# mirage/decompress

Measured on AMD Instinct MI355X. Metric: MiB/s inflate over N zlib streams (uncompressed bytes / wall second), higher is better.
Workload: dtype u8; 1 GPU; C2: 4096 x 256 KiB zlib streams per GPU, dynamic Huffman (libz level 6; even streams = slices of the reference's test/corpus, odd = order-2 Markov ASCII text, 64 symbols, seed 0xC2 + i, SURVEY 8(d)), Zl.Inf.Ns semantics, one stream per pair of wavefronts (decoder + copier); streams_per_gpu=4096, stream_bytes=262144, unique_streams=4096

## Files before the change

decompress_amd/csrc/inflate_wave.hip:

```cpp
#include <stdlib.h>
#include "inflate_util.hpp"
#include "internal.hpp"

namespace md {
namespace wv {

constexpr uint32_t S = 264;
constexpr uint32_t SMIN = 48;
constexpr uint32_t KMAX = 64;
#ifndef MD_EMIT_SPLIT
#define MD_EMIT_SPLIT 1
#endif
#if defined(MD_DEBUG_KNOWN_BOUNDS)
#undef MD_EMIT_SPLIT
#define MD_EMIT_SPLIT 0
#endif
#ifndef MD_SPLIT_B
#define MD_SPLIT_B 4
#endif
#ifndef MD_RUNIN_NUM
#define MD_RUNIN_NUM 3
#define MD_RUNIN_DEN 2
#endif
constexpr uint32_t RUNIN_NUM = MD_RUNIN_NUM, RUNIN_DEN = MD_RUNIN_DEN;
constexpr uint32_t PASSES = 5;
constexpr uint32_t PASS_BITS = 1600, PASSES_MAX = 16;
#ifndef MD_RMAX
#define MD_RMAX 576
#endif
#ifndef MD_STAGE
#define MD_STAGE 5248
#endif
#ifndef MD_PAIR_OCC
#define MD_PAIR_OCC 5
#endif
constexpr uint32_t RMAX = MD_RMAX;
constexpr uint32_t STAGE = MD_STAGE;
constexpr uint32_t WIN_WORDS = 544;

constexpr uint32_t kLitSize = 852, kDistSize = 592;
constexpr uint32_t kLitRootMax = 512;
constexpr uint32_t kLitSubB = 0;
constexpr uint32_t kDistB = kLitSize - kLitRootMax;
constexpr uint32_t kLitB = kDistB + kDistSize;
constexpr uint32_t kStopEobI = kLitB + kLitRootMax;
constexpr uint32_t kStopBadI = kStopEobI + 2;
constexpr uint32_t kLutWords = kStopBadI + 2;
constexpr uint32_t kTbMask = 0xffe00000u;
constexpr uint32_t kLoopy = 0x100u;
static_assert(kDistB % 2 == 0 && kLitB % 2 == 0 && kStopEobI % 2 == 0 && kLutWords == 1448, "even table bases");
constexpr uint32_t kStEob = 100, kStTrunc = 101;
constexpr uint32_t kCountMatch = 1u << 20;
constexpr uint32_t kNearBit = 0x8000u;

struct Mail {
  uint32_t emitted;
  uint32_t copied;
  uint32_t kind;
  uint32_t total;
  uint32_t x;
  uint32_t stuck;
  uint32_t a, b;
};
constexpr uint32_t kJobRound = 0, kJobStored = 1, kJobQuit = 2, kJobEmit = 3;
constexpr uint32_t kHxUni = 4 * 64;
struct Smem {
  uint32_t win[WIN_WORDS];
  uint32_t lut[kLutWords];
  uint32_t mrec[RMAX];
  uint16_t mpos[RMAX];
  alignas(16) uint8_t stage[STAGE + 16];
  uint16_t list[RMAX];
  Mail mail;
};
struct HScratch {
  uint8_t lens[384];
  uint16_t work[320];
  uint32_t ctr;
};
#if MD_RMAX == 576 && MD_STAGE == 5248
static_assert(sizeof(Smem) <= 17920, "9 streams (18 wavefronts) per CU: 160 KiB / 9, in whole 512-byte units");
#endif
static_assert(RMAX % 64 == 0 && STAGE % 16 == 0 && RMAX * 2 >= (kHxUni + 6) * 4, "record rows, staging chunks, the emit job's words in `list`");
constexpr uint32_t kHScratchAt = 1136;
static_assert(kHScratchAt >= 4 + 572 + 8 && kHScratchAt % 16 == 0 && kHScratchAt + sizeof(HScratch) <= WIN_WORDS * 4, "header scratch lives behind the header's bits");
typedef MD_LDS Smem lds_smem;
typedef MD_LDS HScratch lds_hscratch;
__device__ __forceinline__ lds_hscratch *hscratch_of(lds_smem *sm) {
  return reinterpret_cast<lds_hscratch *>(reinterpret_cast<lds_u8 *>(sm->win) + kHScratchAt);
}

#ifdef MD_DEBUG_KNOWN_BOUNDS
constexpr uint32_t KB_ROUNDS = 512;
__device__ uint4 *g_kb_buf;
__device__ int g_kb_mode;
#endif
__device__ __forceinline__ uint32_t mk_entry(uint32_t n, uint32_t xb, uint32_t val8, uint32_t nbits, uint32_t tb) {
  return n | (xb << 5) | (val8 << 9) | (nbits << 17) | (tb << 21);
}
__device__ __forceinline__ uint32_t e_n(uint32_t e) { return e & 31; }
__device__ __forceinline__ uint32_t e_xb(uint32_t e) { return (e >> 5) & 15; }
__device__ __forceinline__ uint32_t e_val(uint32_t e) { return (e >> 9) & 255; }
__device__ __forceinline__ uint32_t e_tb(uint32_t e) { return e >> 21; }
__device__ __forceinline__ bool e_link(uint32_t e) { return e_tb(e) < kLitB && e_tb(e) != kDistB; }
__device__ __forceinline__ uint32_t e_root(uint32_t lroot) { return mk_entry(0, 0, 0, lroot, kLitB); }
__device__ __forceinline__ uint32_t lit_leaf(uint32_t sym, uint32_t codelen, uint32_t lroot, uint32_t droot) {
  if (sym < 256) return mk_entry(codelen, 0, sym, lroot, kLitB);
  if (sym == 256) return mk_entry(codelen, 0, 0, 0, kStopEobI);
  const uint32_t l = (sym - 257) & 31;
  const uint32_t xb = (l >= 8 && l < 28) ? (l - 4) >> 2 : 0;
  const uint32_t base3 = l < 8 ? l : l < 28 ? (4 + (l & 3)) << xb : l == 28 ? 255 : 0;
  return mk_entry(codelen + xb, xb, base3, droot, kDistB);
}
__device__ __forceinline__ uint32_t dist_leaf(uint32_t dv, uint32_t codelen, uint32_t lroot) {
  dv &= 31;
  if (dv >= 30) return mk_entry(codelen, 0, 0, 0, kStopBadI);
  const uint32_t xb = dv >= 4 ? (dv - 2) >> 1 : 0;
  const uint32_t m = dv < 4 ? dv : ((dv & 1) | 2);
  return mk_entry(codelen + xb, xb, m, lroot, kLitB);
}
__device__ __forceinline__ uint32_t dist_value(uint32_t m, uint32_t xb, uint32_t x) { return (m << xb) + 1 + x; }

struct Window {
  uint32_t w[8], wx;
  uint32_t base;
#ifdef MD_DEBUG_KNOWN_BOUNDS
  uint32_t kb_round, kb_sid;
#endif
  __device__ __forceinline__ void fetch(const uint8_t *__restrict__ body, uint32_t nbytes, uint32_t b, uint32_t lane) {
    base = b;
    const uint32_t off = b + lane * 32;
#pragma unroll
    for (int k = 0; k < 8; k++) w[k] = 0;
    if (off + 32 <= nbytes) __builtin_memcpy(w, body + off, 32);
    else if (off < nbytes)
      for (uint32_t k = 0; k < 32 && off + k < nbytes; k++) w[k >> 2] |= (uint32_t)body[off + k] << (8 * (k & 3));
    wx = 0;
    if (lane < WIN_WORDS - 512) {
      const uint32_t ox = b + 2048 + lane * 4;
      if (ox + 4 <= nbytes) __builtin_memcpy(&wx, body + ox, 4);
      else if (ox < nbytes)
        for (uint32_t k = 0; k < 4 && ox + k < nbytes; k++) wx |= (uint32_t)body[ox + k] << (8 * k);
    }
  }
  __device__ __forceinline__ void put(lds_u32 *win, uint32_t lane) const {
    lds_u32 *dst = win + lane * 8;
#pragma unroll
    for (int k = 0; k < 8; k++) dst[k] = w[k];
    if (lane < WIN_WORDS - 512) win[512 + lane] = wx;
  }
  __device__ __forceinline__ void ensure(lds_u32 *win, const uint8_t *__restrict__ body, uint32_t nbytes, uint32_t b, uint32_t lane) {
    if (base != b) fetch(body, nbytes, b, lane);
    put(win, lane);
    base = 0xffffffffu;
  }
};
__device__ __forceinline__ uint32_t peek(const lds_u32 *win, uint32_t p) {
  const lds_u32 *q = reinterpret_cast<const lds_u32 *>(reinterpret_cast<const lds_u8 *>(win) + ((p >> 3) & ~3u));
  return __builtin_amdgcn_alignbit(q[1], q[0], p & 31);
}
__device__ __forceinline__ uint32_t lut_at(const lds_u32 *lut, uint32_t tb, uint32_t idx) {
  return *reinterpret_cast<const lds_u32 *>(reinterpret_cast<const lds_u8 *>(lut) + ((tb + idx) << 2));
}

struct UBits {
  const lds_u32 *win;
  uint64_t buf;
  uint32_t n;
  uint32_t wp;
  __device__ __forceinline__ void init(const lds_u32 *w, uint32_t bp) {
    win = w;
    wp = bp >> 5;
    buf = ((uint64_t)uni(win[wp]) | ((uint64_t)uni(win[wp + 1]) << 32)) >> (bp & 31);
    n = 64 - (bp & 31);
    wp += 2;
  }
  __device__ __forceinline__ uint32_t pos() const { return wp * 32 - n; }
  __device__ __forceinline__ void fill() {
    if (n <= 32) {
      buf |= (uint64_t)uni(win[wp]) << n;
      n += 32;
      wp++;
    }
  }
  __device__ __forceinline__ uint32_t peekb(uint32_t k) const { return (uint32_t)buf & ((1u << k) - 1); }
  __device__ __forceinline__ void drop(uint32_t k) {
    buf >>= k;
    n -= k;
  }
};

struct Canon {
  uint32_t cnt[16];
  uint32_t first[16];
  uint32_t offs[16];
  uint32_t max, min, root, left;
};
__device__ __forceinline__ uint32_t lane_rank(uint64_t m) {
  return __builtin_amdgcn_mbcnt_hi((uint32_t)(m >> 32), __builtin_amdgcn_mbcnt_lo((uint32_t)m, 0));
}
template <int K>
__device__ __forceinline__ void canon_counts(const uint32_t (&len)[K], uint32_t rootpref, Canon &c) {
#pragma unroll
  for (int l = 1; l < 16; l++) {
    uint32_t n = 0;
#pragma unroll
    for (int k = 0; k < K; k++) n += (uint32_t)__builtin_popcountll(__ballot(len[k] == (uint32_t)l));
    c.cnt[l] = n;
  }
  c.cnt[0] = 0;
  c.max = 0;
  c.min = 16;
#pragma unroll
  for (int l = 15; l >= 1; l--) {
    if (c.cnt[l] && c.max == 0) c.max = l;
    if (c.cnt[l]) c.min = l;
  }
  int left = 1;
  bool over = false;
  uint32_t code = 0, off = 0;
  c.first[0] = 0;
  c.offs[0] = 0;
#pragma unroll
  for (int l = 1; l < 16; l++) {
    left = (left << 1) - (int)c.cnt[l];
    over = over || left < 0;
    code = (code + c.cnt[l - 1]) << 1;
    c.first[l] = code;
    c.offs[l] = off;
    off += c.cnt[l];
  }
  c.left = over ? 0xffffffffu : (uint32_t)left;
  uint32_t root = rootpref;
  if (root > c.max) root = c.max;
  if (root < c.min) root = c.min;
  c.root = root;
}

template <int K, class LEAF>
__device__ __forceinline__ bool build_walk(const uint32_t (&len)[K], const Canon &c, lds_u32 *lut, uint32_t tb0, uint32_t sub0,
                                           uint32_t size, lds_hscratch *hs, uint32_t lane, uint32_t zero_entry, LEAF leaf) {
  const uint32_t root = c.root, rmask = (1u << root) - 1;
  uint32_t rev[K];
#pragma unroll
  for (int k = 0; k < K; k++) rev[k] = 0;
#pragma unroll
  for (int l = 1; l < 16; l++) {
    if (c.cnt[l]) {
      uint32_t base = 0;
#pragma unroll
      for (int k = 0; k < K; k++) {
        const uint64_t m = __ballot(len[k] == (uint32_t)l);
        if (len[k] == (uint32_t)l) {
          const uint32_t rank = base + lane_rank(m);
          rev[k] = __brev(c.first[l] + rank) >> (32 - l);
          hs->work[c.offs[l] + rank] = (uint16_t)(lane + 64 * k);
        }
        base += (uint32_t)__builtin_popcountll(m);
      }
    }
  }
  const uint32_t nroot = 1u << root;
  for (uint32_t i = lane; i < nroot; i += kWave) lut[tb0 + i] = 0;
  if (lane == 0) hs->ctr = 0;
  if (c.max > root) {
#pragma unroll
    for (int k = 0; k < K; k++)
      if (len[k] > root)
        __hip_atomic_fetch_max(&lut[tb0 + (rev[k] & rmask)], len[k], __ATOMIC_RELAXED, __HIP_MEMORY_SCOPE_WORKGROUP);
  }
  for (uint32_t i = lane; i < nroot; i += kWave) {
    const uint32_t v = lut[tb0 + i];
    uint32_t e;
    if (v) {
      const uint32_t sub = v - root;
      const uint32_t off = __hip_atomic_fetch_add(&hs->ctr, 1u << sub, __ATOMIC_RELAXED, __HIP_MEMORY_SCOPE_WORKGROUP);
      e = mk_entry(root, 0, 0, sub, (sub0 + off) & 2047);
    } else {
      const uint32_t cw = __brev(i) >> (32 - root);
      uint32_t fl = 0, ft = 0;
#pragma unroll
      for (int l = 15; l >= 1; l--) {
        if (c.cnt[l] && (uint32_t)l <= root) {
          const uint32_t t = (cw >> (root - l)) - c.first[l];
          if (t < c.cnt[l]) {
            fl = l;
            ft = c.offs[l] + t;
          }
        }
      }
      e = fl ? leaf((uint32_t)hs->work[ft], fl) : zero_entry;
    }
    lut[tb0 + i] = e;
  }
  const uint32_t used = nroot + uni(hs->ctr);
  if (used > size) return false;
  if (c.max > root) {
#pragma unroll
    for (int k = 0; k < K; k++) {
      if (len[k] > root) {
        const uint32_t link = lut[tb0 + (rev[k] & rmask)];
        const uint32_t sub = (link >> 17) & 15, tb = link >> 21;
        const uint32_t e = leaf(lane + 64 * k, len[k] - root);
        for (uint32_t j = rev[k] >> root; j < (1u << sub); j += 1u << (len[k] - root)) lut[tb + j] = e;
      }
    }
  }
  return true;
}

constexpr uint64_t kZig0 = 16ull | 17ull << 5 | 18ull << 10 | 0ull << 15 | 8ull << 20 | 7ull << 25 | 9ull << 30 | 6ull << 35 |
                           10ull << 40 | 5ull << 45 | 11ull << 50 | 4ull << 55;
constexpr uint64_t kZig1 = 12ull | 3ull << 5 | 13ull << 10 | 2ull << 15 | 14ull << 20 | 1ull << 25 | 15ull << 30;

template <class PF>
__device__ __noinline__ int dynamic_tables(lds_smem *sm, uint32_t bp_arg, uint32_t tot_arg, uint32_t lane, uint32_t *bp_out,
                                           uint32_t *lroot_out, PF &pf) {
  const uint32_t bp = uni(bp_arg), tot = uni(tot_arg);
  const lds_u32 *win = (const lds_u32 *)sm->win;
  lds_hscratch *hs = hscratch_of(sm);
  UBits ub;
  ub.init(win, bp);
  if ((int32_t)(tot - ub.pos()) < 14) return MD_UNEXPECTED_END_OF_INPUT;
  const uint32_t hlit = ub.peekb(5) + 257;
  ub.drop(5);
  const uint32_t hdist = ub.peekb(5) + 1;
  ub.drop(5);
  const uint32_t hclen = ub.peekb(4) + 4;
  ub.drop(4);
  uint32_t cl[1] = {0};
  for (uint32_t i = 0; i < hclen; i++) {
    ub.fill();
    if ((int32_t)(tot - ub.pos()) < 3) return MD_UNEXPECTED_END_OF_INPUT;
    const uint32_t v = ub.peekb(3);
    ub.drop(3);
    const uint32_t z = (uint32_t)((i < 12 ? kZig0 >> (5 * i) : kZig1 >> (5 * (i - 12))) & 31);
    if (lane == z) cl[0] = v;
  }
  Canon cc;
  canon_counts<1>(cl, 7, cc);
  uint32_t cmaxl, t_lo, t_hi;
  if (cc.max == 0) {
    cmaxl = 1;
    t_lo = lane == 0 ? (1u << 8) : 0xffffu;
    t_hi = 0xffffu;
  } else {
    if (cc.left != 0) return MD_INVALID_DICTIONARY;
    cmaxl = cc.max;
#pragma unroll
    for (int l = 1; l < 8; l++) {
      const uint64_t m = __ballot(cl[0] == (uint32_t)l);
      if (cl[0] == (uint32_t)l) hs->work[cc.offs[l] + lane_rank(m)] = (uint16_t)lane;
    }
    uint32_t t[2];
#pragma unroll
    for (int h = 0; h < 2; h++) {
      const uint32_t i = lane + 64 * h;
      const uint32_t cw = __brev(i & ((1u << cmaxl) - 1)) >> (32 - cmaxl);
      uint32_t fl = 0, ft = 0;
#pragma unroll
      for (int l = 7; l >= 1; l--) {
        if (cc.cnt[l] && (uint32_t)l <= cmaxl) {
          const uint32_t x = (cw >> (cmaxl - l)) - cc.first[l];
          if (x < cc.cnt[l]) {
            fl = l;
            ft = cc.offs[l] + x;
          }
        }
      }
      t[h] = fl ? ((uint32_t)hs->work[ft] | (fl << 8)) : 0xffffu;
    }
    t_lo = t[0];
    t_hi = t[1];
  }
  const uint32_t max_res = hlit + hdist;
  for (uint32_t x = lane; x < 384; x += kWave) hs->lens[x] = 0;
  auto run_lengths = [&](auto checked) -> int {
    constexpr bool CHECK = decltype(checked)::value;
    uint32_t i = 0, prev = 0;
    while (i < max_res) {
      ub.fill();
      if (CHECK && (int32_t)(tot - ub.pos()) < (int32_t)cmaxl) return MD_UNEXPECTED_END_OF_INPUT;
      const uint32_t idx = ub.peekb(cmaxl);
      const uint32_t e_lo = __builtin_amdgcn_readlane(t_lo, idx & 63), e_hi = __builtin_amdgcn_readlane(t_hi, idx & 63);
      const uint32_t e = idx < 64 ? e_lo : e_hi;
      if (e == 0xffffu) return MD_INVALID_DICTIONARY;
      const uint32_t sym = e & 0xff;
      ub.drop(e >> 8);
      if (sym < 16) {
        hs->lens[i] = (uint8_t)sym;
        prev = sym;
        i++;
      } else {
        const uint32_t nb = sym == 16 ? 2 : sym == 17 ? 3 : 7;
        if (sym == 16 && i == 0) return MD_INVALID_DICTIONARY;
        ub.fill();
        if (CHECK && (int32_t)(tot - ub.pos()) < (int32_t)nb) return MD_UNEXPECTED_END_OF_INPUT;
        const uint32_t copy = ub.peekb(nb) + (sym == 18 ? 11 : 3);
        ub.drop(nb);
        const uint32_t val = sym == 16 ? prev : 0;
        if (i + copy > max_res) return MD_INVALID_DICTIONARY;
        if (val)
          for (uint32_t x = lane; x < copy; x += kWave) hs->lens[i + x] = (uint8_t)val;
        prev = val;
        i += copy;
      }
    }
    return MD_OK;
  };
  {
    const bool plenty = (int32_t)(tot - ub.pos()) >= 316 * 14 + 64;
    const int rc = plenty ? run_lengths(std::false_type{}) : run_lengths(std::true_type{});
    if (rc != MD_OK) return rc;
  }
  *bp_out = ub.pos();
  pf.tick_lds(P_HDR_LENS);
  if (uni(hs->lens[256]) == 0) return MD_INVALID_DICTIONARY;
  uint32_t ll[5], dl[1];
#pragma unroll
  for (int k = 0; k < 5; k++) ll[k] = lane + 64 * k < hlit ? (uint32_t)hs->lens[lane + 64 * k] : 0u;
  dl[0] = lane < hdist ? (uint32_t)hs->lens[hlit + lane] : 0u;
  Canon cl_, cd_;
  canon_counts<5>(ll, 9, cl_);
  canon_counts<1>(dl, 6, cd_);
  if (cl_.left == 0xffffffffu || (cl_.left > 0 && cl_.max != 1)) return MD_INVALID_DICTIONARY;
  const uint32_t lroot = cl_.root;
  uint32_t droot;
  lds_u32 *lut = (lds_u32 *)sm->lut;
  if (cd_.max == 0) {
    droot = 1;
  } else {
    if (cd_.left == 0xffffffffu || (cd_.left > 0 && cd_.max != 1)) return MD_INVALID_DICTIONARY;
    droot = cd_.root;
  }
  if (!build_walk<5>(ll, cl_, lut, kLitB, kLitSubB, kLitSize, hs, lane, e_root(lroot),
                     [=](uint32_t sym, uint32_t codelen) { return lit_leaf(sym, codelen, lroot, droot); }))
    return MD_INVALID_DICTIONARY;
  pf.tick_lds(P_HDR_LIT);
  if (cd_.max == 0) {
    if (lane == 0) {
      lut[kDistB] = dist_leaf(0, 1, lroot);
      lut[kDistB + 1] = mk_entry(0, 0, 0, 0, kStopBadI);
    }
  } else if (!build_walk<1>(dl, cd_, lut, kDistB, kDistB + (1u << droot), kDistSize, hs, lane, e_root(lroot),
                            [=](uint32_t sym, uint32_t codelen) { return dist_leaf(sym, codelen, lroot); }))
    return MD_INVALID_DICTIONARY;
  const bool loopy = cl_.left > 0 || (cd_.max != 0 && cd_.left > 0);
  *lroot_out = lroot | (loopy ? kLoopy : 0u);
  return MD_OK;
}

__device__ __noinline__ void fixed_tables(lds_smem *sm, uint32_t lane, uint32_t *lroot_out) {
  lds_hscratch *hs = hscratch_of(sm);
  uint32_t ll[5], dl[1];
#pragma unroll
  for (int k = 0; k < 5; k++) {
    const uint32_t n = lane + 64 * k;
    ll[k] = n < 144 ? 8 : n < 256 ? 9 : n < 280 ? 7 : n < 288 ? 8 : 0;
  }
  dl[0] = lane < 32 ? 5 : 0;
  Canon cl_, cd_;
  canon_counts<5>(ll, 9, cl_);
  canon_counts<1>(dl, 6, cd_);
  const uint32_t lroot = cl_.root, droot = cd_.root;
  lds_u32 *lut = (lds_u32 *)sm->lut;
  build_walk<5>(ll, cl_, lut, kLitB, kLitSubB, kLitSize, hs, lane, e_root(lroot),
                [=](uint32_t sym, uint32_t codelen) { return lit_leaf(sym, codelen, lroot, droot); });
  build_walk<1>(dl, cd_, lut, kDistB, kDistB + (1u << droot), kDistSize, hs, lane, e_root(lroot),
                [=](uint32_t sym, uint32_t codelen) { return dist_leaf(sym, codelen, lroot); });
  *lroot_out = lroot;
}

struct Cursor {
  uint32_t w0, w1, w2, wa;
  __device__ __forceinline__ void init(const lds_u32 *win, uint32_t p) {
    wa = (p >> 5) << 2;
    const lds_u32 *q = reinterpret_cast<const lds_u32 *>(reinterpret_cast<const lds_u8 *>(win) + wa);
    w0 = q[0];
    w1 = q[1];
    w2 = q[2];
  }
  __device__ __forceinline__ uint32_t peek(uint32_t p) const { return __builtin_amdgcn_alignbit(w1, w0, p); }
  __device__ __forceinline__ void seek(const lds_u32 *win, uint32_t pn) {
    const uint32_t wan = (pn >> 5) << 2;
    const bool ge = wan != wa;
    w0 = ge ? w1 : w0;
    w1 = ge ? w2 : w1;
    wa = wan;
    w2 = *reinterpret_cast<const lds_u32 *>(reinterpret_cast<const lds_u8 *>(win) + wa + 8);
  }
};
__device__ __forceinline__ uint32_t lut_step(const lds_u32 *lut, uint32_t e, uint32_t w) {
  return lut_at(lut, e >> 21, __builtin_amdgcn_ubfe(w, 0, e >> 17));
}

template <bool COUNT, bool BUDGET, bool MID = false>
__device__ __forceinline__ void sync_pass(const lds_u32 *win, const lds_u32 *lut, uint32_t lroot, bool go, uint32_t start,
                                          uint32_t limit, uint32_t &end, uint32_t &stop, uint32_t &nb, uint32_t mthr = 0,
                                          uint32_t *midp = nullptr, uint32_t *midcnt = nullptr) {
  if (go) {
    uint32_t p = start, e = e_root(lroot), cnt = 0;
    uint32_t mp = 0xffffffffu, mc = 0;
    bool got = false;
    if (MID && start >= mthr) {
      mp = start;
      got = true;
    }
    if (p < limit) {
      const uint32_t thr = (kLitB << 21) | limit;
      uint32_t slot = 0, key;
      Cursor c;
      c.init(win, start);
      do {
        const uint32_t w = c.peek(p);
        const uint32_t en = lut_step(lut, e, w);
        const uint32_t n = e_n(en);
        if (COUNT) {
          const uint32_t xb = e_xb(en);
          const uint32_t len1 = e_val(en) + __builtin_amdgcn_ubfe(w, n - xb, xb) + (kCountMatch + 2);
          cnt += (e_tb(en) == kLitB ? 1u : 0u) + (e_tb(en) == kDistB ? len1 : 0u);
        }
        p += n;
        if (MID) {
          const bool cross = (e_tb(en) == kLitB) & !got & (p >= mthr);
          mp = cross ? p : mp;
          mc = cross ? cnt : mc;
          got = got | cross;
        }
        c.seek(win, p);
        e = en;
        key = (en & kTbMask) | p;
        if (BUDGET && ++slot >= KMAX && e_tb(en) == kLitB) break;
      } while (key < thr);
    }
    end = p;
    stop = e_tb(e) >= kStopEobI ? e_tb(e) : 0u;
    if (COUNT) nb = cnt;
    if (MID) {
      *midp = mp;
      *midcnt = mc;
    }
  }
}

struct LaneOut {
  uint32_t endp;
  uint32_t stopc;
  uint32_t bytes;
  uint32_t nm;
};

__device__ __noinline__ uint32_t slow_token(const lds_u32 *win, const lds_u32 *lut, uint32_t lroot, uint32_t ptok, uint32_t q,
                                            uint32_t tot, uint32_t cap) {
  uint32_t p = ptok;
  uint32_t w = peek(win, p);
  uint32_t e = lut_step(lut, e_root(lroot), w);
  if (e_link(e)) {
    p += e_n(e);
    w = peek(win, p);
    e = lut_step(lut, e, w);
  }
  uint32_t n = e_n(e), xb = e_xb(e), ntb = e_tb(e);
  uint32_t pn = p + n;
  if (pn > tot) return MD_UNEXPECTED_END_OF_INPUT;
  if (ntb == kStopEobI) return kStEob | (pn << 8);
  if (ntb != kDistB) {
    if (q >= cap) return MD_UNEXPECTED_END_OF_OUTPUT;
    return kStTrunc;
  }
  const uint32_t mlen = e_val(e) + 3 + __builtin_amdgcn_ubfe(w, n - xb, xb);
  p = pn;
  w = peek(win, p);
  e = lut_step(lut, e, w);
  if (e_tb(e) == kStopBadI && e_n(e) == 0) return MD_INVALID_DISTANCE_CODE;
  if (e_link(e)) {
    p += e_n(e);
    w = peek(win, p);
    e = lut_step(lut, e, w);
  }
  n = e_n(e), xb = e_xb(e);
  pn = p + n;
  if (pn > tot) return MD_UNEXPECTED_END_OF_INPUT;
  if (e_tb(e) == kStopBadI) return MD_INVALID_DISTANCE_CODE;
  const uint32_t d = dist_value(e_val(e), xb, __builtin_amdgcn_ubfe(w, n - xb, xb));
  const uint32_t lim = q < 32768u ? q : 32768u;
  if (d > lim) return MD_INVALID_DISTANCE;
  if (mlen > cap - q) return MD_UNEXPECTED_END_OF_OUTPUT;
  return kStTrunc;
}

template <bool CHECKED, bool BUDGET>
__device__ __forceinline__ void emit_pass(const lds_u32 *win, const lds_u32 *lut, uint32_t lroot, lds_u32 *mrec,
                                          lds_u16 *mpos, lds_u8 *stage, uint32_t rec0, uint32_t tot, bool go, uint32_t start,
                                          uint32_t limit, uint32_t q0, uint32_t rb, uint32_t R0, uint32_t cap, LaneOut &lo) {
  uint32_t p = start, ptok = start, e = e_root(lroot);
  uint32_t q = q0, rec = rec0, mlen = 0;
  bool stopped = false;
  const uint32_t qlim = rb + STAGE - 16;
  const uint32_t qmax = cap < qlim ? cap : qlim;
  if (go && p < limit) {
    const uint32_t thr = (kLitB << 21) | limit;
    uint32_t slot = 0, key;
    Cursor c;
    c.init(win, start);
    do {
      const uint32_t w = c.peek(p);
      const uint32_t en = lut_step(lut, e, w);
      const uint32_t n = e_n(en), xb = e_xb(en), ntb = e_tb(en);
      const uint32_t x = __builtin_amdgcn_ubfe(w, n - xb, xb);
      const uint32_t pn = p + n;
      const bool to_root = ntb == kLitB, is_len = ntb == kDistB;
      const bool mat = to_root & (mlen != 0), lit = to_root & (mlen == 0);
      const uint32_t d1 = (e_val(en) << xb) + x;
      if (CHECKED) {
        const uint32_t lim = q < 32768u ? q : 32768u;
        const uint32_t need = mat ? mlen : 1u;
        stopped = (ntb >= kStopEobI) | (pn > tot) | (mat & (d1 >= lim)) | (to_root & (q + need > qmax));
        if (stopped) break;
      }
      stage[lit ? q - rb : STAGE + 15] = (uint8_t)(en >> 9);
      if (mat) {
        mrec[rec] = ((mlen - 3) << 16) | ((q - d1 + mlen > R0 + 1) ? kNearBit : 0u) | d1;
        mpos[rec] = (uint16_t)(q - rb);
        rec++;
      }
      q += to_root ? (mlen > 1u ? mlen : 1u) : 0u;
      mlen = is_len ? e_val(en) + 3 + x : to_root ? 0u : mlen;
      p = pn;
      ptok = to_root ? pn : ptok;
      c.seek(win, p);
      e = en;
      key = (en & kTbMask) | p;
      if (BUDGET && ++slot >= KMAX && to_root) break;
    } while (key < thr);
    if (!CHECKED) stopped = e_tb(e) >= kStopEobI;
  }
  uint32_t stopc = 0, endp = p;
  if (go && stopped) {
    const uint32_t r = slow_token(win, lut, lroot, ptok, q, tot, cap);
    stopc = r & 0xffu;
    endp = stopc == kStEob ? r >> 8 : ptok;
  }
  if (go) {
    lo.endp = endp;
    lo.stopc = stopc;
    lo.bytes = q - q0;
    lo.nm = rec - rec0;
  }
}

struct Sink {
  lds_u8 *stage;
  uint8_t *g;
  uint32_t cap;
  uint32_t pos;
  uint32_t lane;
  uint32_t a, b;
  bool want_adler;
  __device__ __forceinline__ uint32_t sbase() const { return pos & ~15u; }

  __device__ __forceinline__ void flush(uint32_t total) {
    const uint32_t rb = sbase();
    const uint32_t endp = pos + total;
    const uint32_t full0 = (pos + 15) & ~15u, full1 = endp & ~15u;
    uint32_t s1 = 0, s2 = 0;
    for (uint32_t ps = full0; ps < full1; ps += 1024) {
      const uint32_t cpos = ps + lane * 16;
      if (cpos < full1) {
        const lds_u32 *sp = reinterpret_cast<const lds_u32 *>(stage + (cpos - rb));
        const uint32_t w0 = sp[0], w1 = sp[1], w2 = sp[2], w3 = sp[3];
        const uint4 v = make_uint4(w0, w1, w2, w3);
        __builtin_memcpy(g + cpos, &v, 16);
        if (want_adler) {
          uint32_t t1 = __builtin_amdgcn_udot4(w0, 0x01010101u, 0u, false);
          t1 = __builtin_amdgcn_udot4(w1, 0x01010101u, t1, false);
          t1 = __builtin_amdgcn_udot4(w2, 0x01010101u, t1, false);
          t1 = __builtin_amdgcn_udot4(w3, 0x01010101u, t1, false);
          uint32_t tk = __builtin_amdgcn_udot4(w0, 0x03020100u, 0u, false);
          tk = __builtin_amdgcn_udot4(w1, 0x07060504u, tk, false);
          tk = __builtin_amdgcn_udot4(w2, 0x0b0a0908u, tk, false);
          tk = __builtin_amdgcn_udot4(w3, 0x0f0e0d0cu, tk, false);
          s1 += t1;
          s2 += (endp - cpos) * t1 - tk;
        }
      }
    }
    {
      const uint32_t head1 = full0 < endp ? full0 : endp;
      const uint32_t tail0 = full1 > head1 ? full1 : head1;
      const uint32_t x = lane < 16 ? pos + lane : tail0 + (lane - 16);
      if (lane < 16 ? x < head1 : (lane < 32 && x < endp)) {
        const uint32_t d = stage[x - rb];
        g[x] = (uint8_t)d;
        s1 += d;
        s2 += (endp - x) * d;
      }
    }
    if (want_adler) {
      s1 = wave_sum(s1);
      s2 = wave_sum(s2 % 65521u);
      b = (b + total * a + s2) % 65521u;
      a = (a + s1) % 65521u;
    }
    pos = endp;
  }
};

constexpr int FR = RMAX / kWave;
struct FarRow {
  uint32_t qs, n, src;
  bool near, has;
  uint32_t ml;
};
__device__ __forceinline__ FarRow far_row(const lds_u32 *mrec, const lds_u16 *mpos, uint32_t r, uint32_t nrec, uint32_t rb, uint32_t R0) {
  FarRow f;
  f.has = r < nrec;
  const uint32_t tk = mrec[f.has ? r : 0u];
  f.qs = mpos[f.has ? r : 0u];
// ... 849 lines not shown
```

Measured before the change: 249,400 MiB/s.

## Decode code-length symbols lane-parallel per 64-bit window in dynamic header

Adds a wave-parallel decoder for the dynamic Huffman code-length sequence. Each lane speculatively decodes a code-length symbol starting at its own bit offset within a 64-bit window. A readlane chain then follows the true symbol boundaries, and the lengths are written with an exclusive scan plus a broadcast of the previous value for repeat code 16. When it cannot proceed (near end of input, invalid code, or code 16 at index 0), it falls back to the serial decoder from the saved state. It targets the serial per-symbol latency of header parsing, at the cost of extra bpermute and scan work per window.

```diff
diff --git a/decompress_amd/csrc/inflate_wave.hip b/decompress_amd/csrc/inflate_wave.hip
--- a/decompress_amd/csrc/inflate_wave.hip
+++ b/decompress_amd/csrc/inflate_wave.hip
@@ -313,6 +313,62 @@
                            10ull << 40 | 5ull << 45 | 11ull << 50 | 4ull << 55;
 constexpr uint64_t kZig1 = 12ull | 3ull << 5 | 13ull << 10 | 2ull << 15 | 14ull << 20 | 1ull << 25 | 15ull << 30;
 
+struct ClChain {
+  uint32_t pos;
+  uint32_t i;
+  uint32_t prev;
+};
+constexpr uint32_t kClIs16 = 1u << 8, kClBad = 1u << 9;
+__device__ __forceinline__ uint32_t cl_pack(uint32_t skip, uint32_t value, uint32_t count) { return skip | (value << 4) | (count << 24); }
+__device__ __forceinline__ uint32_t cl_skip(uint32_t r) { return r & 15; }
+__device__ __forceinline__ uint32_t cl_value(uint32_t r) { return (r >> 4) & 15; }
+__device__ __forceinline__ uint32_t cl_count(uint32_t r) { return r >> 24; }
+__device__ __forceinline__ bool lengths_by_lane(const lds_u32 *win, lds_hscratch *hs, uint32_t t_lo, uint32_t t_hi, uint32_t cmaxl,
+                                                uint32_t tot, uint32_t max_res, uint32_t lane, ClChain &st) {
+  while (st.i < max_res) {
+    const uint32_t w0 = st.pos & ~63u;
+    if ((int32_t)(tot - w0) < 64 + 14) return false;
+    const uint32_t w = peek(win, w0 + lane);
+    const uint32_t idx = w & ((1u << cmaxl) - 1);
+    const uint32_t e_lo = (uint32_t)__builtin_amdgcn_ds_bpermute((int)((idx & 63) << 2), (int)t_lo);
+    const uint32_t e_hi = (uint32_t)__builtin_amdgcn_ds_bpermute((int)((idx & 63) << 2), (int)t_hi);
+    const uint32_t e = idx < 64 ? e_lo : e_hi;
+    const uint32_t sym = e & 0xff, cl = (e >> 8) & 15;
+    const uint32_t x = w >> cl;
+    const bool rep = sym >= 16;
+    const uint32_t nb = sym == 16 ? 2 : sym == 17 ? 3 : 7;
+    const uint32_t cnt = rep ? (sym == 18 ? 11 : 3) + (x & ((1u << nb) - 1)) : 1;
+    uint32_t pk = cl_pack(cl + (rep ? nb : 0), rep ? 0 : sym, cnt) | (sym == 16 ? kClIs16 : 0);
+    if (e == 0xffffu) pk = cl_pack(15, 0, 0) | kClBad;
+    uint32_t p = st.pos - w0, i = st.i, acc = 0;
+    uint64_t vis = 0;
+    uint32_t r = __builtin_amdgcn_readlane(pk, p);
+    if (i == 0 && (r & kClIs16)) return false;
+    for (;;) {
+      vis |= 1ull << p;
+      acc |= r;
+      p += cl_skip(r);
+      i += cl_count(r);
+      if ((int32_t)((p - 64) & (i - max_res)) >= 0) break;
+      r = __builtin_amdgcn_readlane(pk, p);
+    }
+    if ((acc & kClBad) || i > max_res) return false;
+    const bool v = (vis >> lane) & 1;
+    const uint32_t at = st.i + wave_excl_scan(v ? cl_count(pk) : 0u, lane);
+    const uint64_t sets = vis & ~__ballot((pk & kClIs16) != 0);
+    const uint32_t setv = cl_value(pk);
+    const uint64_t below = sets & ((1ull << lane) - 1);
+    const uint32_t src = below ? 63 - (uint32_t)__builtin_clzll(below) : 0;
+    const uint32_t got = (uint32_t)__builtin_amdgcn_ds_bpermute((int)(src << 2), (int)setv);
+    const uint32_t val = (pk & kClIs16) ? (below ? got : st.prev) : setv;
+    if (v && val) lds_put((lds_u8 *)hs->lens + at, (uint64_t)val * 0x0101010101010101ull, cl_count(pk));
+    if (sets) st.prev = __builtin_amdgcn_readlane(setv, 63 - (uint32_t)__builtin_clzll(sets));
+    st.pos = w0 + p;
+    st.i = i;
+  }
+  return true;
+}
+
 template <class PF>
 __device__ __noinline__ int dynamic_tables(lds_smem *sm, uint32_t bp_arg, uint32_t tot_arg, uint32_t lane, uint32_t *bp_out,
                                            uint32_t *lroot_out, PF &pf) {
@@ -375,9 +431,10 @@
   }
   const uint32_t max_res = hlit + hdist;
   for (uint32_t x = lane; x < 384; x += kWave) hs->lens[x] = 0;
+  ClChain st = {ub.pos(), 0, 0};
   auto run_lengths = [&](auto checked) -> int {
     constexpr bool CHECK = decltype(checked)::value;
-    uint32_t i = 0, prev = 0;
+    uint32_t i = st.i, prev = st.prev;
     while (i < max_res) {
       ub.fill();
       if (CHECK && (int32_t)(tot - ub.pos()) < (int32_t)cmaxl) return MD_UNEXPECTED_END_OF_INPUT;
@@ -408,12 +465,17 @@
     }
     return MD_OK;
   };
-  {
+  uint32_t hend = st.pos;
+  if (lengths_by_lane(win, hs, t_lo, t_hi, cmaxl, tot, max_res, lane, st)) {
+    hend = st.pos;
+  } else {
+    ub.init(win, st.pos);
     const bool plenty = (int32_t)(tot - ub.pos()) >= 316 * 14 + 64;
     const int rc = plenty ? run_lengths(std::false_type{}) : run_lengths(std::true_type{});
     if (rc != MD_OK) return rc;
-  }
-  *bp_out = ub.pos();
+    hend = ub.pos();
+  }
+  *bp_out = uni(hend);
   pf.tick_lds(P_HDR_LENS);
   if (uni(hs->lens[256]) == 0) return MD_INVALID_DICTIONARY;
   uint32_t ll[5], dl[1];
```

Measured after the change: 251,300 MiB/s (median of 6 runs). Within noise of the previous version (+0.8%).
